# aicodix/modem

Measured on AMD Instinct MI355X. Metric: decoded frames/sec + BER, mode-6 8kHz OFDM, batch 65536, 1/2/4/8 MI355X, higher is better.
Workload: dtype f32

## Files before the change

### modem_amd/csrc/api_internal.h

```cpp
#pragma once
#include "../../include/ofdmrx.h"
#include "kernels.h"
#include "tables.h"
#include <hip/hip_runtime.h>
#include <dlfcn.h>
#include <algorithm>
#include <array>
#include <cmath>
#include <cstdio>
#include <cstdlib>
#include <vector>
#include <cstring>
#include <new>
#include <string>
#include <vector>

using namespace rx;


static_assert(sizeof(Result) == sizeof(ofdmrx_frame_result), "Result must mirror ofdmrx_frame_result");
static_assert(sizeof(Attempt) == sizeof(ofdmrx_attempt) && ATTEMPTS_MAX == OFDMRX_MAX_SKIP + 1, "Attempt must mirror ofdmrx_attempt");


extern thread_local std::string g_last_error;
// ... 117 lines not shown
	DevBuf payload[2], res[2];
	DevBuf chunk_flags;
	DevBuf soft;
	DevBuf q_ctl, q_slots, q_llr, q_hard, q_metric, q_lane_mesg;
	unsigned q_cap = 0;
	DevBuf s_ctl, s_slots, s_llr, s_cw, s_xw, s_stat, sc_soft;
	unsigned s_cap = 0;
	unsigned sc_unit = 1;
	int sc_mode = 1;
	int sc_grid = 0, sc_grid6 = 0;
	int sc_top = 1;
	int sc_lb = 6;
	ListQueue *sc_queue() const { return s_ctl.as<ListQueue>(); }
	ScRing sc_ring() const { return sc_mode ? ScRing{ s_ctl.as<ListQueue>(), s_slots.as<ListSlot>(), s_llr.as<float>() } : ScRing{ nullptr, nullptr, nullptr }; }
	unsigned flush_unit = 1;
	DevBuf rot_tap;
	DevBuf tx_code, tx_rowsym, tx_tdom, tx_big;
	hipStream_t stream_b = nullptr;
	hipStream_t stream_fin = nullptr;
	hipStream_t stream_c = nullptr;
	hipError_t sticky = hipSuccess;
	int polar_grid = 0;
	int cert_mode = 1;
	float *esn0_user = nullptr;
	DevBuf esn0_dev[2];
	ofdmrx_attempt *att_user = nullptr;
	int32_t *att_counts_user = nullptr;
	DevBuf att_dev[2], attc_dev[2];
	ListQueue *queue() const { return q_ctl.as<ListQueue>(); }
	DevBuf dc, z;
	long last_spf = 0;
	DevBuf in_stage[2], skip_stage;
	void *out_stage[2] = { nullptr, nullptr };
	size_t out_stage_cap[2] = { 0, 0 };
	DevBuf carr;
	DevBuf sc_scratch;
	int last_n = 0;
	size_t last_first = 0;
	bool last_mono = false;
	FrameBatch last_fb{};
	std::vector<hipEvent_t> ev_pool;
	size_t ev_used = 0;
	struct Span { int stage; size_t a, b; };
	std::vector<Span> spans;
	ofdmrx_timing timing{};
	float sc_ms = 0.f;
// ... 85 lines not shown
```

### modem_amd/csrc/api_pipeline.cpp

```cpp
#include "api_internal.h"

int ensure_events(ofdmrx_handle *h, size_t need)
{
	while (h->ev_pool.size() < need) {
		hipEvent_t e;
		HIP_OK(hipEventCreate(&e));
		h->ev_pool.push_back(e);
	}
	return 0;
}
size_t mark(ofdmrx_handle *h, hipStream_t on)
{
	if (h->ev_used >= h->ev_pool.size()) {
		h->sticky = hipErrorOutOfMemory;
		return 0;
	}
	size_t i = h->ev_used++;
	hipError_t e = hipEventRecord(h->ev_pool[i], on ? on : h->stream);
	if (e != hipSuccess && h->sticky == hipSuccess)
		h->sticky = e;
	return i;
}
static size_t events_per_chunk(int max_skip) { return 32 + 16 * (size_t)(max_skip + 1); }

// ... 11 lines not shown
static int run_front1_rounds(ofdmrx_handle *h, hipStream_t s, FrameBatch fb, int n, const int32_t *d_skip, int max_skip,
	size_t *t_begin, Attempt *d_att, int32_t *d_att_counts, size_t wait_before_sync, size_t *ev_after_sync)
{
	const bool mono = fb.channels == 1;
	SyncState *st = h->st.as<SyncState>();
	cf *z = mono ? h->z.as<cf>() : nullptr;
	const MonoArgs ma = mono_args(h->host.front, mono ? h->dc.as<double>() : nullptr, mono_ck_per_frame(fb.samples_per_frame));
	size_t e0 = mark(h, s);
	if (mono) {
		Range r("ofdmrx:front_end");
		launch_mono_carries(s, h->rate, n, fb, h->host.front, h->dc.as<double>());
		if (!mono_fused(h->rate))
			launch_front_end(s, h->rate, n, fb, ma, z);
	}
	size_t e1 = mark(h, s);
	launch_init_sync(s, n, st, d_skip, h->chunk_flags.as<int>(), d_att_counts);
	size_t last = e1;
	for (int round = 0; round <= max_skip; ++round) {
		if (round == 0 && wait_before_sync != (size_t)-1)
			HIP_OK(hipStreamWaitEvent(s, h->ev_pool[wait_before_sync], 0));
		size_t a = mark(h, s);
		{
			Range r("ofdmrx:sync");
			launch_sync(s, h->rate, n, fb, z, h->dev, st, h->sc_scratch.as<cf>(), ma);
		}
		size_t b = mark(h, s);
		if (round == 0)
			*ev_after_sync = b;
		{
			Range r("ofdmrx:header_osd");
			launch_header(s, h->rate, n, fb, z, ma, h->dev, st, h->hdr_soft.as<int8_t>(), d_att, d_att_counts);
		}
		size_t c = mark(h, s);
		h->spans.push_back({ OFDMRX_T_SYNC, a, b });
		h->spans.push_back({ OFDMRX_T_HEADER, b, c });
		last = c;
	}
	{
		Range r("ofdmrx:demod");
		launch_demod(s, h->rate, n, fb, z, ma, h->dev, st, h->cons.as<cf>(), h->carr.as<cf>());
	}
	size_t d = mark(h, s);
	h->spans.push_back({ OFDMRX_T_DEMOD, last, d });
	h->spans.push_back({ OFDMRX_T_FRONT, e0, e1 });
	*t_begin = e0;
	return front1_done(h, fb, n);
}
// ... 27 lines not shown
			launch_header_sources(s, h->rate, n, sb, h->dev, st, h->hdr_soft.as<int8_t>());
	}
	size_t c = mark(h, s);
	h->spans.push_back({ OFDMRX_T_HEADER, b, c });
	{
		Range r("ofdmrx:demod");
		if (windows)
			launch_demod_bank(s, h->rate, n, wb, h->dev, st, h->cons.as<cf>(), h->carr.as<cf>());
		else
			launch_demod_sources(s, h->rate, n, sb, h->dev, st, h->cons.as<cf>(), h->carr.as<cf>());
	}
	size_t d = mark(h, s);
	h->spans.push_back({ OFDMRX_T_DEMOD, c, d });
	*t_begin = e0;
	return front1_done(h, fb, n);
}

static int run_front2(ofdmrx_handle *h, hipStream_t s, int n)
{
	size_t e4 = mark(h, s);
	{
		Range r("ofdmrx:theil_sen");
		launch_theil_sen(s, n, h->st.as<SyncState>(), h->cons.as<cf>(), demod_forms_cons(h->rate) ? nullptr : h->carr.as<cf>(),
			h->slope.as<float>(), h->yint.as<float>(), h->chunk_flags.as<int>());
	}
	size_t e5 = mark(h, s);
	h->spans.push_back({ OFDMRX_T_THEILSEN, e4, e5 });
	HIP_OK(hipGetLastError());
	return 0;
}

void run_sc_pass(ofdmrx_handle *h, hipStream_t s, int n, bool force, int chunk_seq)
{
	Range r("ofdmrx:sc_path");
	launch_sc_plan(s, h->sc_queue(), h->sc_unit, force ? 1 : 0);
	launch_sc(s, h->sc_lb, std::min(h->sc_grid, (n + 1) / 2), std::min(h->sc_grid6, n), h->sc_queue(), h->s_slots.as<ListSlot>(), h->s_llr.as<float>(),
		h->sc_soft.as<float>(), h->s_cw.as<unsigned long long>(), h->s_xw.as<unsigned long long>(), h->s_stat.as<ScStat>(), h->dev, h->sc_top);
	launch_sc_finish(s, (int)std::min<unsigned>(h->s_cap, (unsigned)n + h->sc_unit), h->sc_queue(), h->s_slots.as<ListSlot>(), h->s_llr.as<float>(), h->s_cw.as<unsigned long long>(),
		h->s_xw.as<unsigned long long>(), h->s_stat.as<ScStat>(), h->dev, h->cfg.descramble, h->queue(), h->q_slots.as<ListSlot>(),
		h->q_llr.as<float>(), h->slot_of.as<int>(), chunk_seq);
	launch_sc_adapt(s, h->sc_queue());
}

static int run_back(ofdmrx_handle *h, hipStream_t s, int par, int n, Result *d_res, float *d_esn0, uint8_t *d_payload,
	uint8_t *payload_later, Result *res_later, bool sc_force, int chunk_seq)
{
	size_t e5 = mark(h, s);
// ... 93 lines not shown

struct PipeHooks {
	virtual ~PipeHooks() {}
	virtual int before_front1(size_t c, FrameBatch *fb, size_t *ready) = 0;
	virtual void dst(size_t c, uint8_t **payload, Result **res) = 0;
	virtual float *esn0(size_t) { return nullptr; }
	virtual void attempts(size_t, Attempt **log, int32_t **counts) { *log = nullptr; *counts = nullptr; }
	virtual int after_front1(size_t, size_t ) { return 0; }
	virtual int after_flush(size_t, hipStream_t ) { return 0; }
	virtual void dst_later(size_t, uint8_t **payload, Result **res) { *payload = nullptr; *res = nullptr; }
	virtual int before_flush(size_t, hipStream_t , hipEvent_t ) { return 0; }
	virtual bool outputs_leave_by_chunk() { return false; }
};

static int run_pipeline(ofdmrx_handle *h, PipeHooks &hooks, const ChunkPlan &plan, FrameBatch batch, const int32_t *d_skip, int max_skip,
	const SyncState *seed, const RecordSources *srcs = nullptr)
{
	const size_t n_chunks = plan.count(), NONE = (size_t)-1;
	int r = ensure_events(h, h->ev_used + n_chunks * events_per_chunk(max_skip) + 8);
	r = r ? r : ensure_capacity(h, (int)plan.largest(), batch.channels == 1, batch.samples_per_frame);
	if (r)
		return r;
	const bool overlap = n_chunks > 1 && !std::getenv("OFDMRX_NO_OVERLAP");
	hipStream_t sa = h->stream, sb = overlap ? h->stream_b : sa, sc = overlap ? h->stream_fin : sa;
	const bool every = hooks.outputs_leave_by_chunk();
	const bool scan_slot = overlap;
	std::vector<size_t> ev_back(n_chunks, NONE), ev_polar(n_chunks, NONE), ev_fin(n_chunks, NONE), ev_out(n_chunks, NONE), t0s(n_chunks, 0);
	launch_queue_reset(sa, h->queue(), h->q_cap);
	if (h->sc_mode)
		launch_queue_reset(sa, h->sc_queue(), h->s_cap);
	auto flush = [&](size_t p, size_t ev_sync_next) -> int {
		const int par = (int)(p & 1);
		if (overlap) {
			HIP_OK(hipStreamWaitEvent(sb, h->ev_pool[ev_back[p]], 0));
			if (ev_sync_next != NONE && scan_slot)
				HIP_OK(hipStreamWaitEvent(sb, h->ev_pool[ev_sync_next], 0));
			if (p >= 2)
				HIP_OK(hipStreamWaitEvent(sb, h->ev_pool[ev_fin[p - 2]], 0));
		}
		int rr = hooks.before_flush(p, sc, h->ev_pool[ev_back[p]]);
		ev_out[p] = mark(h, sc);
		rr = rr ? rr : run_flush(h, sb, sc, par, every || p + 1 == n_chunks, t0s[p], &ev_polar[p]);
		rr = rr ? rr : hooks.after_flush(p, sc);
		ev_fin[p] = mark(h, sc);
		return rr;
	};
// ... 346 lines not shown
```

### modem_amd/csrc/dev_common.h

```cpp
#pragma once
#include <hip/hip_runtime.h>
#include <stdint.h>

#if defined(BACK_WALK) || defined(DEMOD_QA_LDS) || defined(DEMOD_RAW_AHEAD) || defined(DEMOD_SWZ) || defined(DEMOD_TWR_BYTES) || defined(POLAR_NT_LEVEL) || defined(POLAR_WPB) || defined(POLAR_XB1) || defined(POLAR_XB2) || defined(POLAR_XB3) || defined(SYNC_FFT_IN_LDS) || defined(SYNC_PER) || defined(SYNC_SPLIT_8K) || defined(SYNC_SPLIT_ROUNDS) || defined(SYNC_WAVES) || defined(SYNC_WAVES_SPLIT_MONO) || defined(TS_CAP) || defined(TS_MARGIN) || defined(TS_MORE_OCC) || defined(TS_MORE_WAVES_N) || defined(TS_OPEN_MARGIN) || defined(TS_OPEN_NEED) || defined(TS_OWN_ATAN) || defined(TS_ROWS_PER_WG) || defined(TS_UNC_STEPS) || defined(TX_NT_LDS) || defined(TX_TW_GLOBAL)
#error "a frozen tuning macro was passed with -D: edit a patched copy of the source instead (tools/experiments/ts_stage_probe.py shows how)"
#endif

namespace rx {

template <int RATE> struct RateCfg {
	static constexpr int SL = (int)((1280L * RATE) / 8000);
	static constexpr int FILTER_LEN = (((21 * RATE) / 8000) & ~3) | 1;
	static constexpr int GL = SL / 8;
	static constexpr int STRIDE = SL + GL;
	static constexpr int HS = SL / 2;
	static constexpr int BUFFER_LEN = 6 * STRIDE;
	static constexpr int SEARCH_POS = BUFFER_LEN - 4 * STRIDE;
	static constexpr int MATCH_LEN = GL | 1;
	static constexpr int MATCH_DEL = (MATCH_LEN - 1) / 2;
};
inline bool rate_supported(int rate) { return rate == 8000 || rate == 16000 || rate == 44100 || rate == 48000; }
inline int rate_symbol_len(int rate) { return (int)((1280L * rate) / 8000); }
inline int rate_filter_len(int rate) { return (((21 * rate) / 8000) & ~3) | 1; }
#define RX_RATE_SWITCH(rate, ...) \
	switch (rate) { \
	case 16000: { constexpr int RATE = 16000; __VA_ARGS__; } break; \
	case 44100: { constexpr int RATE = 44100; __VA_ARGS__; } break; \
// ... 418 lines not shown
	for (int t = 0; t < 4; ++t)
		v[t] = buf[sl + t * 64];
	Bfly<4>::run(v);
	#pragma unroll
	for (int k = 1; k < 4; ++k)
		v[k] = cmul(v[k], twl[(k - 1) * 64 + lane]);
	fft256_transpose<5, 4>(v, lane);
	Bfly<4>::run(v);
	#pragma unroll
	for (int k = 1; k < 4; ++k)
		v[k] = cmul(v[k], twl[(3 + k - 1) * 64 + lane]);
	fft256_transpose<3, 2>(v, lane);
	Bfly<4>::run(v);
	#pragma unroll
	for (int k = 1; k < 4; ++k)
		v[k] = cmul(v[k], twl[(6 + k - 1) * 64 + lane]);
	fft256_transpose<1, 0>(v, lane);
	Bfly<4>::run(v);
	fft_sync<64>();
	#pragma unroll
	for (int t = 0; t < 4; ++t)
		buf[lane + t * 64] = v[t];
	fft_sync<64>();
}

__device__ __forceinline__ long uniform_l(long v)
{
	const int lo = __builtin_amdgcn_readfirstlane((int)v), hi = __builtin_amdgcn_readfirstlane((int)(v >> 32));
	return ((long)hi << 32) | (long)(unsigned)lo;
}
__device__ __forceinline__ float uniform_f(float v) { return __int_as_float(__builtin_amdgcn_readfirstlane(__float_as_int(v))); }
__device__ __forceinline__ double shfl_d(double v, int src)
{
	int lo = __double2loint(v), hi = __double2hiint(v);
	lo = __shfl(lo, src);
	hi = __shfl(hi, src);
	return __hiloint2double(hi, lo);
}
__device__ __forceinline__ double shfl_up_d(double v, int d)
{
	int lo = __double2loint(v), hi = __double2hiint(v);
	lo = __shfl_up(lo, d);
	hi = __shfl_up(hi, d);
	return __hiloint2double(hi, lo);
}
__device__ __forceinline__ double shfl_xor_d(double v, int m)
// ... 207 lines not shown
```

### modem_amd/csrc/k_sync.hip

```cpp
#include <type_traits>
#include "dev_common.h"
#include "kernels.h"
#include "mono_front.h"
#include "sync_accept.h"

#pragma clang fp contract(off)

namespace rx {

constexpr int FE_PER = 16, FE_TILE = 256 * FE_PER, CAR_TB = 6;

template <int RATE>
__global__ __launch_bounds__(256) void k_mono_carries(FrameBatch fb, FrontCoef co, double *__restrict__ ck_all, int ck_per_frame)
{
	const int f = blockIdx.x, tid = threadIdx.x, lane = tid & 63, wave = tid >> 6;
	const long n = fb.samples_per_frame;
	const char *base = (const char *)fb.samples + (size_t)f * fb.frame_stride_bytes;
	MonoFrame fr{ base, fb.fmt, n, nullptr };
	double *ck = ck_all + (size_t)f * ck_per_frame;
	__shared__ double wave_end[CAR_TB][4];
	const double a = (double)co.dc_a, g = (double)co.dc_b * (1.0 - a) * (double)fr.scale();
	double Apow[7];
	Apow[0] = mono_pow(a, FE_PER);
	#pragma unroll
// ... 181 lines not shown
	for (int m = 32; m; m >>= 1)
		nx = fmaxf(nx, __shfl_xor(nx, m));
	const float peak = fmaxf(pk, 0.f);
	const int shift = peak > 0.f ? sh_i : 0;
	if (peak <= nx * 4.f)
		return false;
	cf v = cconj(buf[shift]);
	int pos_err = (int)nearbyintf(atan2f(v.im, v.re) * (float)HALF_LEN / TWO_PI_F);
	if (abs(pos_err) > GUARD_LEN / 2)
		return false;
	symbol_pos -= pos_err;
	float cfo_rad = (float)shift * (TWO_PI_F / (float)HALF_LEN) - frac_cfo;
	if (cfo_rad >= PI_F)
		cfo_rad -= TWO_PI_F;
	symbol_pos_out = symbol_pos;
	cfo_out = cfo_rad;
	return true;
}

struct NoShared {};
#define SYNC_WAVES_SPLIT_MONO 3
template <int RATE, bool SPLIT, bool MONO>
__global__ __launch_bounds__(64, SPLIT ? (MONO ? SYNC_WAVES_SPLIT_MONO : SYNC_WAVES_SPLIT) : SYNC_WAVES) void k_sync(FrameBatch fb, cf *__restrict__ z_all, const cf *__restrict__ tw,
	const cf *__restrict__ kern, SyncState *__restrict__ st_all, cf *__restrict__ scratch, MonoArgs ma)
{
	typedef RateCfg<RATE> RC;
	constexpr int BUFFER_LEN = RC::BUFFER_LEN, SEARCH_POS = RC::SEARCH_POS, HALF_LEN = RC::HS, GUARD_LEN = RC::GL;
	constexpr int MATCH_LEN = RC::MATCH_LEN, MATCH_DEL = RC::MATCH_DEL;
	constexpr int MRING = SyncRing<RATE>::N;
	static_assert(TILE + MATCH_LEN <= MRING, "m ring too small");
	const int f = blockIdx.x, lane = threadIdx.x;
	SyncState st = st_all[f];
	const long n = fb.samples_per_frame;
	if (!st.active || st.found || st.t_next >= n)
		return;
	SampleSrc src{ (const char *)fb.samples + (size_t)f * fb.frame_stride_bytes, fb.fmt, fb.channels, n,
		fb.channels == 1 ? z_all + (size_t)f * fb.samples_per_frame : nullptr };
	__shared__ SyncShared<RATE, SPLIT> sh;
	__shared__ std::conditional_t<MONO, typename MonoCover<RATE, 64>::Shared, NoShared> msh;
	MonoCover<RATE, 64> mc;
	constexpr int D = BUFFER_LEN - 1 - (SEARCH_POS + HALF_LEN);
	if constexpr (MONO)
		mc.init(mono_frame(fb, ma.ck, ma.ck_per_frame, f), ma, &msh, z_all + (size_t)f * fb.samples_per_frame, lane);
	auto need = [&](long p_lo, long p_hi) {
		if constexpr (MONO) {
			mc.cover(ma, p_lo, p_hi, lane);
			__syncthreads();
// ... 2 lines not shown
	cf *fbuf = SYNC_FFT_LDS(RATE) && !SPLIT ? sh.buf : scratch + (size_t)f * 2 * HALF_LEN;
	cf *fxr = SYNC_FFT_LDS(RATE) && !SPLIT ? sh.xr : scratch + (size_t)f * 2 * HALF_LEN + HALF_LEN;
	for (int i = lane; i < MRING + MRING / 8; i += 64)
		sh.m[i] = 0.f;
	const float thr_lo = (float)(0.17 * MATCH_LEN), thr_hi = (float)(0.19 * MATCH_LEN);
	const float min_R = 0.0001f * HALF_LEN;
	const long t_start = st.t_next;
	long T0 = t_start - (MATCH_LEN - 1);
	constexpr long FIRST = D - HALF_LEN;
	if (T0 < FIRST - (MATCH_LEN - 1)) T0 = FIRST - (MATCH_LEN - 1);
	double Wr = 0.0, Wi = 0.0, Wp = 0.0, Wm = 0.0;
	if (T0 > FIRST) {
		need(T0 - 1 - D - (HALF_LEN - 1), T0 - D + HALF_LEN);
		direct_P<RATE>(src, T0 - 1, lane, Wr, Wi);
		Wp = direct_R<RATE>(src, T0 - 1, lane);
	}
	bool collecting = false, found = false, pending = false;
	float tmax = 0.f;
	long nmax = 0;
	int rejects = st.rejects;
	__syncthreads();
	for (; T0 < n && !found && !pending; T0 += TILE) {
		double dr[PER], di[PER], dp[PER];
		{
			const long tb = T0 + lane * PER;
			auto phase1 = [&](auto at) {
				#pragma unroll
				for (int e = 0; e < PER; ++e) {
					long a = tb + e - (BUFFER_LEN - 1 - (SEARCH_POS + HALF_LEN));
					cf zA = at(a - HALF_LEN), zB = at(a), zC = at(a + HALF_LEN);
					double inr = (double)zB.re * zC.re + (double)zB.im * zC.im;
					double ini = (double)zB.im * zC.re - (double)zB.re * zC.im;
					double outr = (double)zA.re * zB.re + (double)zA.im * zB.im;
					double outi = (double)zA.im * zB.re - (double)zA.re * zB.im;
					double pin = (double)zC.re * zC.re + (double)zC.im * zC.im;
					double pout = (double)zA.re * zA.re + (double)zA.im * zA.im;
					double pr = inr - outr, pi = ini - outi, pp = pin - pout;
					dr[e] = (e ? dr[e - 1] : 0.0) + pr;
					di[e] = (e ? di[e - 1] : 0.0) + pi;
					dp[e] = (e ? dp[e - 1] : 0.0) + pp;
				}
			};
			const long w_lo = T0 - (BUFFER_LEN - 1 - (SEARCH_POS + HALF_LEN)) - HALF_LEN, w_hi = w_lo + TILE + 2 * HALF_LEN;
			if constexpr (MONO) {
				if (!mc.any || mc.next < w_hi)
					need(w_lo, w_hi);
				else
					__syncthreads();
				mc.cover(ma, w_lo, w_hi + TILE, lane);
			}
			if (src.mode() == 1 && w_lo >= 0 && w_hi <= n) {
				const short2 *p = (const short2 *)src.base;
				phase1([&](long i) { const short2 v = p[i]; return mk(div_32767((float)v.x), div_32767((float)v.y)); });
			} else if (MONO && w_lo >= 0 && w_hi <= n) {
				const cf *p = src.analytic;
				phase1([&](long i) { return p[i]; });
			} else if (src.mode() == 1 && w_hi <= n) {
				const short2 *p = (const short2 *)src.base;
				phase1([&](long i) {
					const short2 v = p[i < 0 ? 0 : i];
					return i < 0 ? mk(0.f, 0.f) : mk(div_32767((float)v.x), div_32767((float)v.y));
				});
			} else if (MONO && w_hi <= n) {
				const cf *p = src.analytic;
				phase1([&](long i) { const cf v = p[i < 0 ? 0 : i]; return i < 0 ? mk(0.f, 0.f) : v; });
			} else {
				phase1([&](long i) { return src.at(i); });
			}
		}
		double or_ = wave_scan_incl(dr[PER - 1], lane) - dr[PER - 1] + Wr;
		double oi_ = wave_scan_incl(di[PER - 1], lane) - di[PER - 1] + Wi;
		double op_ = wave_scan_incl(dp[PER - 1], lane) - dp[PER - 1] + Wp;
		#pragma unroll
		for (int e = 0; e < PER; ++e) {
			float Pre = (float)(or_ + dr[e]), Pim = (float)(oi_ + di[e]);
			float R = 0.5f * (float)(op_ + dp[e]);
			R = fmaxf(R, min_R);
			const float mf = __fdiv_rn(__fadd_rn(__fmul_rn(Pre, Pre), __fmul_rn(Pim, Pim)), __fmul_rn(R, R));
			sh.m[sync_pad((int)((T0 + lane * PER + e) & (MRING - 1)))] = mf;
		}
		Wr = shfl_d(or_ + dr[PER - 1], 63);
		Wi = shfl_d(oi_ + di[PER - 1], 63);
		Wp = shfl_d(op_ + dp[PER - 1], 63);
		__syncthreads();
		double dm[PER];
		#pragma unroll
		for (int e = 0; e < PER; ++e) {
			long t = T0 + lane * PER + e;
			double in = (double)sh.m[sync_pad((int)(t & (MRING - 1)))];
			double out = (t - MATCH_LEN >= 0) ? (double)sh.m[sync_pad((int)((t - MATCH_LEN) & (MRING - 1)))] : 0.0;
			dm[e] = (e ? dm[e - 1] : 0.0) + (in - out);
		}
		double om = wave_scan_incl(dm[PER - 1], lane) - dm[PER - 1] + Wm;
		#pragma unroll
		for (int e = 0; e < PER; ++e)
			sh.timing[sync_pad(lane * PER + e)] = (float)(om + dm[e]);
		Wm = shfl_d(om + dm[PER - 1], 63);
		__syncthreads();
		long cur = T0 > t_start ? T0 : t_start;
		long tile_end = T0 + TILE < n ? T0 + TILE : n;
		while (cur < tile_end && !found && !pending) {
			if (!collecting) {
				int fr = first_index(sh.timing, (int)T0, lane, (int)cur, (int)tile_end, true, thr_hi);
				if (fr == 0x7fffffff)
					break;
				collecting = true;
				cur = fr;
// ... 35 lines not shown
			tmax = 0.f;
			if constexpr (SPLIT) {
				pending = true;
				st.pend_g = g;
				st.pend_index_max = index_max;
				st.pend_phase = phase_max;
				st.t_next = (long)g + 1;
			} else {
				int sp;
				float cfo;
				need((long)g - (BUFFER_LEN - 1) + (SEARCH_POS - index_max) + HALF_LEN, (long)g - (BUFFER_LEN - 1) + (SEARCH_POS - index_max) + 2 * HALF_LEN);
				if (sc_process<RATE>(fbuf, fxr, src, tw, kern, g, index_max, phase_max, lane, sp, cfo)) {
					found = true;
					st.symbol_pos = sp;
					st.cfo_rad = cfo;
					st.sc_start = (long)g - (BUFFER_LEN - 1) + sp;
					st.t_next = (long)g + 1;
				} else {
					++rejects;
				}
			}
			cur = (long)g + 1;
		}
		__syncthreads();
	}
	st.rejects = rejects;
	st.found = found ? 1 : 0;
	st.pending = pending ? 1 : 0;
	if (!found && !pending)
		st.t_next = n;
	if (lane == 0)
		st_all[f] = st;
}

template <int RATE, bool MONO>
__global__ __launch_bounds__(256) void k_sync_accept(FrameBatch fb, cf *__restrict__ z_all, const cf *__restrict__ tw,
	const cf *__restrict__ kern, SyncState *__restrict__ st_all, MonoArgs ma)
{
	typedef RateCfg<RATE> RC;
	constexpr int BUFFER_LEN = RC::BUFFER_LEN, SEARCH_POS = RC::SEARCH_POS, HALF_LEN = RC::HS, NT = 256;
	const int f = blockIdx.x, tid = threadIdx.x, lane = tid & 63, wave = tid >> 6;
	SyncState st = st_all[f];
	if (!st.active || st.found || !st.pending)
		return;
	const long n = fb.samples_per_frame;
	SampleSrc src{ (const char *)fb.samples + (size_t)f * fb.frame_stride_bytes, fb.fmt, fb.channels, n,
// ... 79 lines not shown
{
	const int stretches = (int)((fb.samples_per_frame + FE_STRETCH - 1) / FE_STRETCH);
	for (int f0 = 0; f0 < n; f0 += 65535) {
		const int nf = n - f0 < 65535 ? n - f0 : 65535;
		FrameBatch fbq = fb;
		fbq.samples = (const char *)fb.samples + (size_t)f0 * fb.frame_stride_bytes;
		MonoArgs maq = ma;
		maq.ck = ma.ck + (size_t)f0 * ma.ck_per_frame;
		RX_RATE_SWITCH(rate, hipLaunchKernelGGL(k_front_end<RATE>, dim3(stretches, nf), dim3(256), 0, s, fbq, maq, z + (size_t)f0 * fb.samples_per_frame));
	}
}
void launch_streams_front(hipStream_t s, int rate, int n_src, long max_len, SourceBatch fb, MonoArgs ma, cf *z)
{
	const unsigned stretches = (unsigned)((max_len + FE_STRETCH - 1) / FE_STRETCH);
	RX_RATE_SWITCH(rate, hipLaunchKernelGGL((k_front_end<RATE, SourceBatch>), dim3(stretches, (unsigned)n_src), dim3(256), 0, s, fb, ma, z));
}
long front_end_stretch() { return FE_STRETCH; }
void launch_bank_front_end(hipStream_t s, int rate, int n_ch, long max_stretch, WindowBatch fb, MonoArgs ma, cf *z)
{
	RX_RATE_SWITCH(rate, hipLaunchKernelGGL((k_front_end<RATE, WindowBatch>), dim3((unsigned)max_stretch, (unsigned)n_ch), dim3(256), 0, s, fb, ma, z));
}
#define SYNC_SPLIT_ROUNDS 2
template <int RATE, bool MONO>
static void sync_rounds(hipStream_t s, int n, FrameBatch fb, cf *z, Tables tb, SyncState *st, cf *scratch, const MonoArgs &ma)
{
#define SYNC_SPLIT_8K 1
	if (RATE != 8000 || SYNC_SPLIT_8K) {
		for (int r = 0; r < SYNC_SPLIT_ROUNDS; ++r) {
			hipLaunchKernelGGL((k_sync<RATE, true, MONO>), dim3(n), dim3(64), 0, s, fb, z, tb.tw_sym, tb.sc_kern, st, scratch, ma);
			hipLaunchKernelGGL((k_sync_accept<RATE, MONO>), dim3(n), dim3(256), 0, s, fb, z, tb.tw_sym, tb.sc_kern, st, ma);
		}
	}
	hipLaunchKernelGGL((k_sync<RATE, false, MONO>), dim3(n), dim3(64), 0, s, fb, z, tb.tw_sym, tb.sc_kern, st, scratch, ma);
}
void launch_sync(hipStream_t s, int rate, int n, FrameBatch fb, cf *z, Tables tb, SyncState *st, cf *scratch, const MonoArgs &ma)
{
	if (fb.channels == 1 && mono_fused(rate)) {
		sync_rounds<8000, true>(s, n, fb, z, tb, st, scratch, ma);
	} else {
		RX_RATE_SWITCH(rate, (sync_rounds<RATE, false>(s, n, fb, z, tb, st, scratch, ma)));
	}
}

}
```

### modem_amd/csrc/k_theilsen.hip

```cpp
#include "dev_common.h"
#include "kernels.h"

namespace rx {

#define TS_CAP 56
#define TS_OPEN_NEED 30
#define TS_OPEN_MARGIN 6
#define TS_MARGIN 12
#define TS_UNC_STEPS 24
constexpr int TS_QBITS = 22;
constexpr uint32_t TS_QREAL = (1u << TS_QBITS) - 8192u;
constexpr uint32_t TS_QPAD0 = (1u << TS_QBITS) - 4096u;
constexpr uint32_t TS_MQ = 2;
constexpr int TS_MQ1S = (int)((TS_MQ + 1) << 9);
constexpr int TS_LIST = 64;
constexpr int TS_MAX_IT = 48;
constexpr uint32_t TS_SENTINEL = 0x7fffffffu;

constexpr int TS_YS = 68, TS_PS = 76;
#define TS_ROWS_PER_WG 1
#define TS_SYNC() __syncthreads()
struct TsLds {
	float y[8 * TS_YS];
	uint2 sk[8 * TS_PS];
// ... 620 lines not shown
	if (mod_bits == 3) {
		p = -5.951132927e-02f;
		p = fmaf(p, z, 1.054106507e-01f);
		p = fmaf(p, z, -1.423576012e-01f);
		p = fmaf(p, z, 1.999798680e-01f);
		p = fmaf(p, z, -3.333330347e-01f);
		p = fmaf(p, z, 9.999999993e-01f);
	} else {
		p = -1.718391760e-03f;
		p = fmaf(p, z, 1.059115275e-02f);
		p = fmaf(p, z, -3.059610274e-02f);
		p = fmaf(p, z, 5.738879400e-02f);
		p = fmaf(p, z, -8.370542419e-02f);
		p = fmaf(p, z, 1.094069024e-01f);
		p = fmaf(p, z, -1.426187097e-01f);
		p = fmaf(p, z, 1.999827962e-01f);
		p = fmaf(p, z, -3.333328490e-01f);
		p = fmaf(p, z, 9.999999978e-01f);
	}
	return p * t;
}

__device__ __forceinline__ void ts_row(TsLds &s, int f, int j, int lane, const ModeDesc &md, cf *__restrict__ cons_all,
	const cf *__restrict__ carr_all, float *__restrict__ slope_all, float *__restrict__ yint_all)
{
	const int cols = md.cols;
	cf *row = cons_all + (size_t)f * CONS_MAX + (size_t)j * cols;
	const cf *cr = carr_all ? carr_all + (size_t)f * CARR_MAX + (size_t)j * cols : nullptr;
	cf pt[8], pv[8];
	#pragma unroll
	for (int q = 0; q < 8; ++q) {
		const int i = lane + 64 * q;
		if (i < cols) {
			if (cr) {
				pt[q] = cr[cols + i];
				pv[q] = cr[i];
			} else
				pt[q] = row[i];
		}
	}
	#pragma unroll
	for (int q = 0; q < 8; ++q) {
		const int i = lane + 64 * q;
		if (i < cols) {
			cf c = pt[q];
			if (cr) {
				c = demod_or_erase(pt[q], pv[q]);
				row[i] = c;
			}
			cf d = cmul(c, cconj(md.mod_bits == 3 ? psk8_hard_map(c) : psk4_hard_map(c)));
			s.y[ts_yaddr(i)] = ts_phase(d, md.mod_bits);
		}
	}
	TS_SYNC();
	const float2 sy = theil_sen_wave(s, cols, lane);
	if (lane == 0) {
		slope_all[(size_t)f * ROWS_MAX + j] = sy.x;
		yint_all[(size_t)f * ROWS_MAX + j] = sy.y;
	}
}

#define TS_MORE_WAVES_N 20480
#define TS_MORE_OCC 5
constexpr int TS_ROWS_DIRECT = 50, TS_MORE_WAVES = TS_MORE_WAVES_N;
__global__ __launch_bounds__(64 * TS_ROWS_PER_WG, 5) void k_theil_sen(const SyncState *__restrict__ st_all, cf *__restrict__ cons_all,
	const cf *__restrict__ carr_all, float *__restrict__ slope_all, float *__restrict__ yint_all, int n_frames, int *__restrict__ chunk_flags)
{
	const int unit = (int)blockIdx.x * TS_ROWS_PER_WG + ((int)threadIdx.x >> 6);
	const int f = __builtin_amdgcn_readfirstlane(unit / TS_ROWS_DIRECT), j = __builtin_amdgcn_readfirstlane(unit % TS_ROWS_DIRECT), lane = threadIdx.x & 63;
	if (f >= n_frames || !st_all[f].okay)
		return;
	const ModeDesc md = mode_desc(st_all[f].oper_mode);
	if (j == 0 && lane == 0 && md.rows > TS_ROWS_DIRECT)
		atomicMax(chunk_flags, md.rows);
	if (j >= md.rows)
		return;
	__shared__ TsLds s_all[TS_ROWS_PER_WG];
	ts_row(s_all[threadIdx.x >> 6], f, j, lane, md, cons_all, carr_all, slope_all, yint_all);
}
__global__ __launch_bounds__(64, TS_MORE_OCC) void k_theil_sen_more(const SyncState *__restrict__ st_all, cf *__restrict__ cons_all,
	const cf *__restrict__ carr_all, float *__restrict__ slope_all, float *__restrict__ yint_all, int n_frames, const int *__restrict__ chunk_flags)
{
	const int more = chunk_flags[0] - TS_ROWS_DIRECT;
	if (more <= 0)
		return;
	const int lane = threadIdx.x, units = n_frames * more;
	__shared__ TsLds s;
	for (int u = (int)blockIdx.x; u < units; u += TS_MORE_WAVES) {
		const int f = u / more, j = TS_ROWS_DIRECT + u % more;
		if (!st_all[f].okay)
			continue;
		const ModeDesc md = mode_desc(st_all[f].oper_mode);
		if (j >= md.rows)
			continue;
		__syncthreads();
		ts_row(s, f, j, lane, md, cons_all, carr_all, slope_all, yint_all);
	}
}
__global__ __launch_bounds__(64 * TS_ROWS_PER_WG, 5) void k_theil_sen_raw(int cols, int rows, const float *__restrict__ y, float *__restrict__ slope_all,
	float *__restrict__ yint_all)
{
	const int r = __builtin_amdgcn_readfirstlane((int)blockIdx.x * TS_ROWS_PER_WG + ((int)threadIdx.x >> 6)), lane = threadIdx.x & 63;
	if (r >= rows)
		return;
	__shared__ TsLds s_all[TS_ROWS_PER_WG];
	TsLds &s = s_all[threadIdx.x >> 6];
	for (int i = lane; i < cols; i += 64)
		s.y[ts_yaddr(i)] = y[(size_t)r * cols + i];
	TS_SYNC();
	const float2 sy = theil_sen_wave(s, cols, lane);
	if (lane == 0) { slope_all[r] = sy.x; yint_all[r] = sy.y; }
}

void launch_theil_sen(hipStream_t s, int n, const SyncState *st, cf *cons, const cf *carr, float *slope, float *yint, int *chunk_flags)
{
	hipLaunchKernelGGL(k_theil_sen, dim3((n * TS_ROWS_DIRECT + TS_ROWS_PER_WG - 1) / TS_ROWS_PER_WG), dim3(64 * TS_ROWS_PER_WG), 0, s, st, cons, carr,
		slope, yint, n, chunk_flags);
	hipLaunchKernelGGL(k_theil_sen_more, dim3(TS_MORE_WAVES), dim3(64), 0, s, st, cons, carr, slope, yint, n,
		chunk_flags);
}
void launch_theil_sen_raw(hipStream_t s, int rows, int cols, const float *y, float *slope, float *yint)
{
	hipLaunchKernelGGL(k_theil_sen_raw, dim3((rows + TS_ROWS_PER_WG - 1) / TS_ROWS_PER_WG), dim3(64 * TS_ROWS_PER_WG), 0, s, cols, rows, y, slope, yint);
}

}
```

### modem_amd/csrc/kernels.h

```cpp
#pragma once
#include <hip/hip_runtime.h>
#include <stdint.h>
#include "dev_common.h"

namespace rx {

struct FrameBatch {
	const void *samples;
	size_t frame_stride_bytes;
	long samples_per_frame;
	int fmt;
	int channels;
};

struct SourceBatch : FrameBatch {
	const int *src_of;
	const int *src_len;
	const long long *tile0;
	const long long *given0;
};
struct WindowBatch : FrameBatch {
	const int *src_of;
	const long long *org;
	const long long *len;
// ... 122 lines not shown

struct Result {
	int32_t status;
	int32_t symbol_pos;
	int64_t sc_start;
	float cfo_rad, cfo_fine, sfo_slope;
	int32_t oper_mode;
	uint64_t call_sign;
	int32_t best_lane, bit_flips;
	float esn0_db_last;
	int32_t n_sync_rejects;
};

struct Attempt {
	int32_t status, symbol_pos;
	float cfo_rad;
	int32_t oper_mode;
	uint64_t call_sign;
};
constexpr int ATTEMPTS_MAX = 65;

void launch_mono_carries(hipStream_t s, int rate, int n, FrameBatch fb, FrontCoef co, double *ck);
void launch_front_end(hipStream_t s, int rate, int n, FrameBatch fb, MonoArgs ma, cf *z);
void launch_sync(hipStream_t s, int rate, int n, FrameBatch fb, cf *z, Tables tb, SyncState *st, cf *scratch, const MonoArgs &ma);
void launch_header(hipStream_t s, int rate, int n, FrameBatch fb, cf *z, const MonoArgs &ma, Tables tb, SyncState *st, int8_t *hdr_soft,
	Attempt *attempts = nullptr, int32_t *attempt_counts = nullptr);
void launch_osd_only(hipStream_t s, int n, Tables tb, const int8_t *soft, uint8_t *hard, int32_t *unique);
bool demod_forms_cons(int rate);
void launch_demod(hipStream_t s, int rate, int n, FrameBatch fb, cf *z, const MonoArgs &ma, Tables tb, const SyncState *st, cf *cons, cf *carr);
void launch_header_sources(hipStream_t s, int rate, int n, SourceBatch fb, Tables tb, SyncState *st, int8_t *hdr_soft);
void launch_demod_sources(hipStream_t s, int rate, int n, SourceBatch fb, Tables tb, const SyncState *st, cf *cons, cf *carr);
void launch_header_bank(hipStream_t s, int rate, int n, WindowBatch fb, Tables tb, SyncState *st, int8_t *hdr_soft);
void launch_demod_bank(hipStream_t s, int rate, int n, WindowBatch fb, Tables tb, const SyncState *st, cf *cons, cf *carr);
void launch_theil_sen(hipStream_t s, int n, const SyncState *st, cf *cons, const cf *carr, float *slope, float *yint, int *chunk_flags);
void launch_theil_sen_raw(hipStream_t s, int rows, int cols, const float *y, float *slope, float *yint);
void launch_back(hipStream_t s, int rate, int n, int cert_mode, const SyncState *st, const cf *cons, const float *slope, const float *yint,
	float *precision, Result *res, float *esn0_rows, Tables tb, int descramble, uint8_t *payload, ListQueue *q, ListSlot *slots,
	float *llr_q, int *slot_of, uint8_t *payload_later = nullptr, Result *res_later = nullptr, ScRing sc = ScRing{ nullptr, nullptr, nullptr }, int chunk_seq = 0);
void launch_rotate_tap(hipStream_t s, const SyncState *st, const cf *cons, const float *slope, const float *yint, cf *out);
void launch_queue_reset(hipStream_t s, ListQueue *q, unsigned cap);
void launch_queue_snap(hipStream_t s, ListQueue *q, int par);
void launch_queue_plan(hipStream_t s, ListQueue *q, int par, unsigned unit, int force);
void launch_queue_fill(hipStream_t s, ListQueue *q, ListSlot *slots, int n, uint8_t *payload, Result *res, int oper_mode);
void launch_sc_plan(hipStream_t s, ListQueue *qs, unsigned unit = 0, int force = 1);
void launch_sc(hipStream_t s, int lb, int grid5, int grid6, ListQueue *qs, const ListSlot *slots, const float *llr_q, float *soft, unsigned long long *cw_q,
	unsigned long long *xw_q, ScStat *stat_q, Tables tb, int top_skip = 1);
void launch_sc_finish(hipStream_t s, int max_entries, ListQueue *qs, const ListSlot *slots_s, const float *llr_s, const unsigned long long *cw_q,
	const unsigned long long *xw_q, const ScStat *stat_q, Tables tb, int descramble, ListQueue *ql, ListSlot *slots_l, float *llr_l, int *slot_of, int chunk_seq = 0);
void launch_sc_adapt(hipStream_t s, ListQueue *qs);
size_t sc_store_bytes(int lb);
int sc_codewords_per_wave(int lb);
void launch_polar(hipStream_t s, int list, int grid, ListQueue *q, int par, const ListSlot *slots, const float *llr_q, float *soft, uint8_t *hard_q,
	Tables tb, float *metric_q);
void launch_finish(hipStream_t s, int list, int max_entries, const ListQueue *q, int par, const ListSlot *slots, const float *llr_q,
	const uint8_t *hard_q, Tables tb, int descramble, uint8_t *lane_mesg_q, int lane_mesg_stride);
void launch_fft_debug(hipStream_t s, int rate, int n, int len, int sign, const cf *in, cf *out, Tables tb);
void launch_awgn_tile(hipStream_t s, const int16_t *base, size_t n_base, int16_t *out, size_t n_out,
// ... 205 lines not shown
```

Measured before the change: 1.854 million.

## Add L2 prefetch touches in sync scan and Theil-Sen kernels

Adds an inline-asm global load helper that touches cache lines of data a later workgroup or tile will read. The split sync kernel prefetches the next tile's PCM window, and the Theil-Sen kernels prefetch the constellation row another wave will process. The aim is to hide DRAM latency behind compute. Theil-Sen occupancy is raised from 5 to 6 waves per SIMD. The cost is extra loads, one more waitcnt per iteration, and an env switch to turn the touches off.

```diff
diff --git a/modem_amd/csrc/api_internal.h b/modem_amd/csrc/api_internal.h
--- a/modem_amd/csrc/api_internal.h
+++ b/modem_amd/csrc/api_internal.h
@@ -163,6 +163,7 @@
 	hipError_t sticky = hipSuccess;
 	int polar_grid = 0;
 	int cert_mode = 1;
+	bool touch = true;
 	float *esn0_user = nullptr;
 	DevBuf esn0_dev[2];
 	ofdmrx_attempt *att_user = nullptr;
diff --git a/modem_amd/csrc/api_pipeline.cpp b/modem_amd/csrc/api_pipeline.cpp
--- a/modem_amd/csrc/api_pipeline.cpp
+++ b/modem_amd/csrc/api_pipeline.cpp
@@ -57,7 +57,7 @@
 		size_t a = mark(h, s);
 		{
 			Range r("ofdmrx:sync");
-			launch_sync(s, h->rate, n, fb, z, h->dev, st, h->sc_scratch.as<cf>(), ma);
+			launch_sync(s, h->rate, n, fb, z, h->dev, st, h->sc_scratch.as<cf>(), ma, h->touch);
 		}
 		size_t b = mark(h, s);
 		if (round == 0)
@@ -131,7 +131,7 @@
 	{
 		Range r("ofdmrx:theil_sen");
 		launch_theil_sen(s, n, h->st.as<SyncState>(), h->cons.as<cf>(), demod_forms_cons(h->rate) ? nullptr : h->carr.as<cf>(),
-			h->slope.as<float>(), h->yint.as<float>(), h->chunk_flags.as<int>());
+			h->slope.as<float>(), h->yint.as<float>(), h->chunk_flags.as<int>(), h->touch);
 	}
 	size_t e5 = mark(h, s);
 	h->spans.push_back({ OFDMRX_T_THEILSEN, e4, e5 });
@@ -271,6 +271,7 @@
 	if (r)
 		return r;
 	const bool overlap = n_chunks > 1 && !std::getenv("OFDMRX_NO_OVERLAP");
+	h->touch = !std::getenv("OFDMRX_NO_TOUCH");
 	hipStream_t sa = h->stream, sb = overlap ? h->stream_b : sa, sc = overlap ? h->stream_fin : sa;
 	const bool every = hooks.outputs_leave_by_chunk();
 	const bool scan_slot = overlap;
diff --git a/modem_amd/csrc/dev_common.h b/modem_amd/csrc/dev_common.h
--- a/modem_amd/csrc/dev_common.h
+++ b/modem_amd/csrc/dev_common.h
@@ -2,7 +2,7 @@
 #include <hip/hip_runtime.h>
 #include <stdint.h>
 
-#if defined(BACK_WALK) || defined(DEMOD_QA_LDS) || defined(DEMOD_RAW_AHEAD) || defined(DEMOD_SWZ) || defined(DEMOD_TWR_BYTES) || defined(POLAR_NT_LEVEL) || defined(POLAR_WPB) || defined(POLAR_XB1) || defined(POLAR_XB2) || defined(POLAR_XB3) || defined(SYNC_FFT_IN_LDS) || defined(SYNC_PER) || defined(SYNC_SPLIT_8K) || defined(SYNC_SPLIT_ROUNDS) || defined(SYNC_WAVES) || defined(SYNC_WAVES_SPLIT_MONO) || defined(TS_CAP) || defined(TS_MARGIN) || defined(TS_MORE_OCC) || defined(TS_MORE_WAVES_N) || defined(TS_OPEN_MARGIN) || defined(TS_OPEN_NEED) || defined(TS_OWN_ATAN) || defined(TS_ROWS_PER_WG) || defined(TS_UNC_STEPS) || defined(TX_NT_LDS) || defined(TX_TW_GLOBAL)
+#if defined(BACK_WALK) || defined(DEMOD_QA_LDS) || defined(DEMOD_RAW_AHEAD) || defined(DEMOD_SWZ) || defined(DEMOD_TWR_BYTES) || defined(POLAR_NT_LEVEL) || defined(POLAR_WPB) || defined(POLAR_XB1) || defined(POLAR_XB2) || defined(POLAR_XB3) || defined(SYNC_FFT_IN_LDS) || defined(SYNC_PER) || defined(SYNC_SPLIT_8K) || defined(SYNC_SPLIT_ROUNDS) || defined(SYNC_WAVES) || defined(SYNC_WAVES_SPLIT_MONO) || defined(TS_CAP) || defined(TS_MARGIN) || defined(TS_MORE_OCC) || defined(TS_MORE_WAVES_N) || defined(TS_OPEN_MARGIN) || defined(TS_OPEN_NEED) || defined(TS_OWN_ATAN) || defined(TS_ROWS_PER_WG) || defined(TS_TOUCH_GROUPS) || defined(TS_UNC_STEPS) || defined(TX_NT_LDS) || defined(TX_TW_GLOBAL)
 #error "a frozen tuning macro was passed with -D: edit a patched copy of the source instead (tools/experiments/ts_stage_probe.py shows how)"
 #endif
 
@@ -467,6 +467,19 @@
 	for (int t = 0; t < 4; ++t)
 		buf[lane + t * 64] = v[t];
 	fft_sync<64>();
+}
+
+__device__ __forceinline__ uint32_t l2_touch(const void *base, uint32_t off)
+{
+	uint32_t sink;
+	const uint64_t b = (uint64_t)base;
+	const uint64_t ub = ((uint64_t)(uint32_t)__builtin_amdgcn_readfirstlane((int)(b >> 32)) << 32) | (uint32_t)__builtin_amdgcn_readfirstlane((int)b);
+	asm volatile("s_nop 4\n\tglobal_load_dword %0, %1, %2" : "=v"(sink) : "v"(off), "s"(ub) : "memory");
+	return sink;
+}
+__device__ __forceinline__ void l2_touch_retire(uint32_t &sink)
+{
+	asm volatile("s_waitcnt vmcnt(0)" : "+v"(sink));
 }
 
 __device__ __forceinline__ long uniform_l(long v)
diff --git a/modem_amd/csrc/k_sync.hip b/modem_amd/csrc/k_sync.hip
--- a/modem_amd/csrc/k_sync.hip
+++ b/modem_amd/csrc/k_sync.hip
@@ -1,5 +1,6 @@
 #include <type_traits>
 #include "dev_common.h"
+#include "touch_plan.h"
 #include "kernels.h"
 #include "mono_front.h"
 #include "sync_accept.h"
@@ -227,7 +228,7 @@
 #define SYNC_WAVES_SPLIT_MONO 3
 template <int RATE, bool SPLIT, bool MONO>
 __global__ __launch_bounds__(64, SPLIT ? (MONO ? SYNC_WAVES_SPLIT_MONO : SYNC_WAVES_SPLIT) : SYNC_WAVES) void k_sync(FrameBatch fb, cf *__restrict__ z_all, const cf *__restrict__ tw,
-	const cf *__restrict__ kern, SyncState *__restrict__ st_all, cf *__restrict__ scratch, MonoArgs ma)
+	const cf *__restrict__ kern, SyncState *__restrict__ st_all, cf *__restrict__ scratch, MonoArgs ma, int touch)
 {
 	typedef RateCfg<RATE> RC;
 	constexpr int BUFFER_LEN = RC::BUFFER_LEN, SEARCH_POS = RC::SEARCH_POS, HALF_LEN = RC::HS, GUARD_LEN = RC::GL;
@@ -276,6 +277,8 @@
 	__syncthreads();
 	for (; T0 < n && !found && !pending; T0 += TILE) {
 		double dr[PER], di[PER], dp[PER];
+		uint32_t sink = 0;
+		bool touch_tile = false;
 		{
 			const long tb = T0 + lane * PER;
 			auto phase1 = [&](auto at) {
@@ -306,6 +309,7 @@
 			if (src.mode() == 1 && w_lo >= 0 && w_hi <= n) {
 				const short2 *p = (const short2 *)src.base;
 				phase1([&](long i) { const short2 v = p[i]; return mk(div_32767((float)v.x), div_32767((float)v.y)); });
+				touch_tile = true;
 			} else if (MONO && w_lo >= 0 && w_hi <= n) {
 				const cf *p = src.analytic;
 				phase1([&](long i) { return p[i]; });
@@ -315,12 +319,14 @@
 					const short2 v = p[i < 0 ? 0 : i];
 					return i < 0 ? mk(0.f, 0.f) : mk(div_32767((float)v.x), div_32767((float)v.y));
 				});
+				touch_tile = true;
 			} else if (MONO && w_hi <= n) {
 				const cf *p = src.analytic;
 				phase1([&](long i) { const cf v = p[i < 0 ? 0 : i]; return i < 0 ? mk(0.f, 0.f) : v; });
 			} else {
 				phase1([&](long i) { return src.at(i); });
 			}
+
 		}
 		double or_ = wave_scan_incl(dr[PER - 1], lane) - dr[PER - 1] + Wr;
 		double oi_ = wave_scan_incl(di[PER - 1], lane) - di[PER - 1] + Wi;
@@ -337,6 +343,13 @@
 		Wi = shfl_d(oi_ + di[PER - 1], 63);
 		Wp = shfl_d(op_ + dp[PER - 1], 63);
 		__syncthreads();
+		if constexpr (SPLIT && !MONO) {
+			if (touch && touch_tile) {
+				const TouchRange ahead = touch_plan_scan(T0, TILE, D, HALF_LEN, n);
+				if (lane < touch_lanes(ahead))
+					sink = l2_touch((const char *)src.base + ahead.off, (uint32_t)touch_lane_off(ahead, lane));
+			}
+		}
 		double dm[PER];
 		#pragma unroll
 		for (int e = 0; e < PER; ++e) {
@@ -418,6 +431,8 @@
 			}
 			cur = (long)g + 1;
 		}
+		if constexpr (SPLIT && !MONO)
+			l2_touch_retire(sink);
 		__syncthreads();
 	}
 	st.rejects = rejects;
@@ -543,24 +558,24 @@
 }
 #define SYNC_SPLIT_ROUNDS 2
 template <int RATE, bool MONO>
-static void sync_rounds(hipStream_t s, int n, FrameBatch fb, cf *z, Tables tb, SyncState *st, cf *scratch, const MonoArgs &ma)
+static void sync_rounds(hipStream_t s, int n, FrameBatch fb, cf *z, Tables tb, SyncState *st, cf *scratch, const MonoArgs &ma, bool touch)
 {
 #define SYNC_SPLIT_8K 1
 	if (RATE != 8000 || SYNC_SPLIT_8K) {
 		for (int r = 0; r < SYNC_SPLIT_ROUNDS; ++r) {
-			hipLaunchKernelGGL((k_sync<RATE, true, MONO>), dim3(n), dim3(64), 0, s, fb, z, tb.tw_sym, tb.sc_kern, st, scratch, ma);
+			hipLaunchKernelGGL((k_sync<RATE, true, MONO>), dim3(n), dim3(64), 0, s, fb, z, tb.tw_sym, tb.sc_kern, st, scratch, ma, touch ? 1 : 0);
 			hipLaunchKernelGGL((k_sync_accept<RATE, MONO>), dim3(n), dim3(256), 0, s, fb, z, tb.tw_sym, tb.sc_kern, st, ma);
 		}
 	}
-	hipLaunchKernelGGL((k_sync<RATE, false, MONO>), dim3(n), dim3(64), 0, s, fb, z, tb.tw_sym, tb.sc_kern, st, scratch, ma);
-}
-void launch_sync(hipStream_t s, int rate, int n, FrameBatch fb, cf *z, Tables tb, SyncState *st, cf *scratch, const MonoArgs &ma)
+	hipLaunchKernelGGL((k_sync<RATE, false, MONO>), dim3(n), dim3(64), 0, s, fb, z, tb.tw_sym, tb.sc_kern, st, scratch, ma, 0);
+}
+void launch_sync(hipStream_t s, int rate, int n, FrameBatch fb, cf *z, Tables tb, SyncState *st, cf *scratch, const MonoArgs &ma, bool touch)
 {
 	if (fb.channels == 1 && mono_fused(rate)) {
-		sync_rounds<8000, true>(s, n, fb, z, tb, st, scratch, ma);
+		sync_rounds<8000, true>(s, n, fb, z, tb, st, scratch, ma, touch);
 	} else {
-		RX_RATE_SWITCH(rate, (sync_rounds<RATE, false>(s, n, fb, z, tb, st, scratch, ma)));
-	}
-}
-
-}
+		RX_RATE_SWITCH(rate, (sync_rounds<RATE, false>(s, n, fb, z, tb, st, scratch, ma, touch)));
+	}
+}
+
+}
diff --git a/modem_amd/csrc/k_theilsen.hip b/modem_amd/csrc/k_theilsen.hip
--- a/modem_amd/csrc/k_theilsen.hip
+++ b/modem_amd/csrc/k_theilsen.hip
@@ -1,5 +1,6 @@
 #include "dev_common.h"
 #include "kernels.h"
+#include "touch_plan.h"
 
 namespace rx {
 
@@ -666,7 +667,7 @@
 }
 
 __device__ __forceinline__ void ts_row(TsLds &s, int f, int j, int lane, const ModeDesc &md, cf *__restrict__ cons_all,
-	const cf *__restrict__ carr_all, float *__restrict__ slope_all, float *__restrict__ yint_all)
+	const cf *__restrict__ carr_all, float *__restrict__ slope_all, float *__restrict__ yint_all, const TouchRange &ahead)
 {
 	const int cols = md.cols;
 	cf *row = cons_all + (size_t)f * CONS_MAX + (size_t)j * cols;
@@ -696,8 +697,12 @@
 			s.y[ts_yaddr(i)] = ts_phase(d, md.mod_bits);
 		}
 	}
+	uint32_t sink = 0;
+	if (lane < touch_lanes(ahead))
+		sink = l2_touch((const char *)cons_all + ahead.off, (uint32_t)touch_lane_off(ahead, lane));
 	TS_SYNC();
 	const float2 sy = theil_sen_wave(s, cols, lane);
+	l2_touch_retire(sink);
 	if (lane == 0) {
 		slope_all[(size_t)f * ROWS_MAX + j] = sy.x;
 		yint_all[(size_t)f * ROWS_MAX + j] = sy.y;
@@ -707,8 +712,10 @@
 #define TS_MORE_WAVES_N 20480
 #define TS_MORE_OCC 5
 constexpr int TS_ROWS_DIRECT = 50, TS_MORE_WAVES = TS_MORE_WAVES_N;
-__global__ __launch_bounds__(64 * TS_ROWS_PER_WG, 5) void k_theil_sen(const SyncState *__restrict__ st_all, cf *__restrict__ cons_all,
-	const cf *__restrict__ carr_all, float *__restrict__ slope_all, float *__restrict__ yint_all, int n_frames, int *__restrict__ chunk_flags)
+#define TS_TOUCH_GROUPS 128
+static_assert(TS_ROWS_DIRECT * COLS_MAX <= CONS_MAX, "touch_plan_ts: any row below TS_ROWS_DIRECT of any row length lies inside the frame's block");
+__global__ __launch_bounds__(64 * TS_ROWS_PER_WG, 6) void k_theil_sen(const SyncState *__restrict__ st_all, cf *__restrict__ cons_all,
+	const cf *__restrict__ carr_all, float *__restrict__ slope_all, float *__restrict__ yint_all, int n_frames, int *__restrict__ chunk_flags, int touch)
 {
 	const int unit = (int)blockIdx.x * TS_ROWS_PER_WG + ((int)threadIdx.x >> 6);
 	const int f = __builtin_amdgcn_readfirstlane(unit / TS_ROWS_DIRECT), j = __builtin_amdgcn_readfirstlane(unit % TS_ROWS_DIRECT), lane = threadIdx.x & 63;
@@ -720,10 +727,11 @@
 	if (j >= md.rows)
 		return;
 	__shared__ TsLds s_all[TS_ROWS_PER_WG];
-	ts_row(s_all[threadIdx.x >> 6], f, j, lane, md, cons_all, carr_all, slope_all, yint_all);
+	const TouchRange ahead = touch && !carr_all ? touch_plan_ts(f * TS_ROWS_DIRECT + j, n_frames, TS_ROWS_DIRECT, md.cols, TS_TOUCH_GROUPS, CONS_MAX) : TouchRange{ 0, 0 };
+	ts_row(s_all[threadIdx.x >> 6], f, j, lane, md, cons_all, carr_all, slope_all, yint_all, ahead);
 }
 __global__ __launch_bounds__(64, TS_MORE_OCC) void k_theil_sen_more(const SyncState *__restrict__ st_all, cf *__restrict__ cons_all,
-	const cf *__restrict__ carr_all, float *__restrict__ slope_all, float *__restrict__ yint_all, int n_frames, const int *__restrict__ chunk_flags)
+	const cf *__restrict__ carr_all, float *__restrict__ slope_all, float *__restrict__ yint_all, int n_frames, const int *__restrict__ chunk_flags, int touch)
 {
 	const int more = chunk_flags[0] - TS_ROWS_DIRECT;
 	if (more <= 0)
@@ -738,7 +746,8 @@
 		if (j >= md.rows)
 			continue;
 		__syncthreads();
-		ts_row(s, f, j, lane, md, cons_all, carr_all, slope_all, yint_all);
+		const TouchRange ahead = touch && !carr_all ? touch_plan_ts_more(__builtin_amdgcn_readfirstlane(u), n_frames, TS_ROWS_DIRECT, more, md.cols, TS_MORE_WAVES, CONS_MAX) : TouchRange{ 0, 0 };
+		ts_row(s, f, j, lane, md, cons_all, carr_all, slope_all, yint_all, ahead);
 	}
 }
 __global__ __launch_bounds__(64 * TS_ROWS_PER_WG, 5) void k_theil_sen_raw(int cols, int rows, const float *__restrict__ y, float *__restrict__ slope_all,
@@ -756,12 +765,12 @@
 	if (lane == 0) { slope_all[r] = sy.x; yint_all[r] = sy.y; }
 }
 
-void launch_theil_sen(hipStream_t s, int n, const SyncState *st, cf *cons, const cf *carr, float *slope, float *yint, int *chunk_flags)
+void launch_theil_sen(hipStream_t s, int n, const SyncState *st, cf *cons, const cf *carr, float *slope, float *yint, int *chunk_flags, bool touch)
 {
 	hipLaunchKernelGGL(k_theil_sen, dim3((n * TS_ROWS_DIRECT + TS_ROWS_PER_WG - 1) / TS_ROWS_PER_WG), dim3(64 * TS_ROWS_PER_WG), 0, s, st, cons, carr,
-		slope, yint, n, chunk_flags);
+		slope, yint, n, chunk_flags, touch ? 1 : 0);
 	hipLaunchKernelGGL(k_theil_sen_more, dim3(TS_MORE_WAVES), dim3(64), 0, s, st, cons, carr, slope, yint, n,
-		chunk_flags);
+		chunk_flags, touch ? 1 : 0);
 }
 void launch_theil_sen_raw(hipStream_t s, int rows, int cols, const float *y, float *slope, float *yint)
 {
diff --git a/modem_amd/csrc/kernels.h b/modem_amd/csrc/kernels.h
--- a/modem_amd/csrc/kernels.h
+++ b/modem_amd/csrc/kernels.h
@@ -168,7 +168,7 @@
 
 void launch_mono_carries(hipStream_t s, int rate, int n, FrameBatch fb, FrontCoef co, double *ck);
 void launch_front_end(hipStream_t s, int rate, int n, FrameBatch fb, MonoArgs ma, cf *z);
-void launch_sync(hipStream_t s, int rate, int n, FrameBatch fb, cf *z, Tables tb, SyncState *st, cf *scratch, const MonoArgs &ma);
+void launch_sync(hipStream_t s, int rate, int n, FrameBatch fb, cf *z, Tables tb, SyncState *st, cf *scratch, const MonoArgs &ma, bool touch);
 void launch_header(hipStream_t s, int rate, int n, FrameBatch fb, cf *z, const MonoArgs &ma, Tables tb, SyncState *st, int8_t *hdr_soft,
 	Attempt *attempts = nullptr, int32_t *attempt_counts = nullptr);
 void launch_osd_only(hipStream_t s, int n, Tables tb, const int8_t *soft, uint8_t *hard, int32_t *unique);
@@ -178,7 +178,7 @@
 void launch_demod_sources(hipStream_t s, int rate, int n, SourceBatch fb, Tables tb, const SyncState *st, cf *cons, cf *carr);
 void launch_header_bank(hipStream_t s, int rate, int n, WindowBatch fb, Tables tb, SyncState *st, int8_t *hdr_soft);
 void launch_demod_bank(hipStream_t s, int rate, int n, WindowBatch fb, Tables tb, const SyncState *st, cf *cons, cf *carr);
-void launch_theil_sen(hipStream_t s, int n, const SyncState *st, cf *cons, const cf *carr, float *slope, float *yint, int *chunk_flags);
+void launch_theil_sen(hipStream_t s, int n, const SyncState *st, cf *cons, const cf *carr, float *slope, float *yint, int *chunk_flags, bool touch);
 void launch_theil_sen_raw(hipStream_t s, int rows, int cols, const float *y, float *slope, float *yint);
 void launch_back(hipStream_t s, int rate, int n, int cert_mode, const SyncState *st, const cf *cons, const float *slope, const float *yint,
 	float *precision, Result *res, float *esn0_rows, Tables tb, int descramble, uint8_t *payload, ListQueue *q, ListSlot *slots,
diff --git a/modem_amd/csrc/touch_plan.h b/modem_amd/csrc/touch_plan.h
--- /dev/null
+++ b/modem_amd/csrc/touch_plan.h
@@ -0,0 +1,68 @@
+#pragma once
+#include <stdint.h>
+#if defined(__HIPCC__)
+#define TOUCH_HD __host__ __device__
+#else
+#define TOUCH_HD
+#endif
+
+namespace rx {
+
+constexpr int TOUCH_LINE = 128;
+constexpr int TOUCH_XCDS = 8;
+constexpr int TOUCH_POINT_BYTES = 8, TOUCH_PCM_BYTES = 4;
+
+struct TouchRange {
+	long long off;
+	int bytes;
+};
+TOUCH_HD inline int touch_lanes(const TouchRange &r) { return r.bytes > 0 ? (r.bytes + TOUCH_LINE - 1) / TOUCH_LINE + 1 : 0; }
+TOUCH_HD inline int touch_lane_off(const TouchRange &r, int lane)
+{
+	const int o = lane * TOUCH_LINE;
+	return o < r.bytes - 4 ? o : r.bytes - 4;
+}
+
+TOUCH_HD inline TouchRange touch_plan_ts(int u, int n_frames, int rows_direct, int cols, int G, int frame_elems)
+{
+	const TouchRange none = { 0, 0 };
+	if (u < 0 || G < 1 || cols < 1 || rows_direct < 1)
+		return none;
+	const long long v = (long long)u + (long long)TOUCH_XCDS * G, units = (long long)n_frames * rows_direct;
+	if (v >= units || units > 0x7fffffffLL)
+		return none;
+	const int f = (int)v / rows_direct, j = (int)v % rows_direct;
+	if ((long long)(j + 1) * cols > frame_elems)
+		return none;
+	const TouchRange r = { ((long long)f * frame_elems + (long long)j * cols) * TOUCH_POINT_BYTES, cols * TOUCH_POINT_BYTES };
+	return r;
+}
+TOUCH_HD inline TouchRange touch_plan_ts_more(int u, int n_frames, int rows_direct, int more, int cols, int stride, int frame_elems)
+{
+	const TouchRange none = { 0, 0 };
+	if (u < 0 || more < 1 || cols < 1 || stride < 1)
+		return none;
+	const long long v = (long long)u + stride, units = (long long)n_frames * more;
+	if (v >= units || units > 0x7fffffffLL)
+		return none;
+	const int f = (int)v / more, j = rows_direct + (int)v % more;
+	if ((long long)(j + 1) * cols > frame_elems)
+		return none;
+	const TouchRange r = { ((long long)f * frame_elems + (long long)j * cols) * TOUCH_POINT_BYTES, cols * TOUCH_POINT_BYTES };
+	return r;
+}
+
+TOUCH_HD inline TouchRange touch_plan_scan(long long T0, int tile, int D, int half_len, long long n)
+{
+	const TouchRange none = { 0, 0 };
+	if (tile < 1 || T0 + tile >= n)
+		return none;
+	const long long w_hi = T0 - D + half_len + tile;
+	const long long lo = w_hi < 0 ? 0 : w_hi, hi = w_hi + tile < n ? w_hi + tile : n;
+	if (lo >= hi)
+		return none;
+	const TouchRange r = { lo * TOUCH_PCM_BYTES, (int)(hi - lo) * TOUCH_PCM_BYTES };
+	return r;
+}
+
+}
```

Result: no change. 1.859 million, median of 2 (+0.3%).
